# interpreting-video-features/interpreting-video-features

Hardware: AMD Instinct MI355X
Metric: clips/sec full mask-search (I3D, 16f, 300 iters) (higher is better)
Workload: dtype f32 (each operand as 3 bf16 planes = 24 significand bits, 6 MFMA passes, f32 accumulate, f32 storage); 1 GPU; I3D perturbation mask search, 300 iters, synthetic clips [32,3,16,224,224] per GPU per step (BASELINE configs[1]); init_mask + search + reverse score + Grad-CAM; iters=300, frames=16, math=bf16x6

## Files before the change

### interpreting-video-features_amd/csrc/conv3d.hip

```cpp
#include "conv_common.h"

namespace ivf {

template <int BM, int BN, int WM, int WN>
__global__ __launch_bounds__(256) void conv3d_igemm_kernel(ConvKArgs a) {
  constexpr int TM = BM / WM / 32;
  constexpr int TN = BN / WN / 32;
  constexpr int AROWS = BM / 32;
  constexpr int BROWS = BN / 32;
  static_assert(WM * WN == 4, "4 waves");
  static_assert(TM >= 1 && TN >= 1, "tile");

  __shared__ __attribute__((aligned(16))) float lds_a[BM * LDS_LD];
  __shared__ __attribute__((aligned(16))) float lds_b[BN * LDS_LD];

  const int tid = threadIdx.x;
  const int lane = tid & 63;
  const int wave = tid >> 6;
  const int wm = wave / WN, wn = wave % WN;
  const int li = lane & 31, lh = lane >> 5;

  const int tile = xcd_remap(blockIdx.x, a.mtiles * a.ntiles);
  const int mt = tile / a.ntiles;
  const int nt = tile - mt * a.ntiles;
  const int m0 = mt * BM;
  const int n0 = nt * BN;

  const int g = tid & 7;
  const int r0 = tid >> 3;

  int a_base[AROWS];
  int a_t0[AROWS], a_h0[AROWS], a_w0[AROWS];
#pragma unroll
  for (int j = 0; j < AROWS; ++j) {
    int m = m0 + r0 + 32 * j;
    if (m < a.M) {
      int wo = m % a.Wo;
      int t1 = m / a.Wo;
      int ho = t1 % a.Ho;
      int t2 = t1 / a.Ho;
      int to = t2 % a.To;
      int b = t2 / a.To;
      a_t0[j] = to * a.sT - a.pT;
      a_h0[j] = ho * a.sH - a.pH;
      a_w0[j] = wo * a.sW - a.pW;
      a_base[j] = b * a.Ti;
    } else {
      a_t0[j] = -100000;
      a_h0[j] = 0;
      a_w0[j] = 0;
      a_base[j] = 0;
    }
  }
  const float* wrow[BROWS];
#pragma unroll
  for (int j = 0; j < BROWS; ++j) {
    int n = n0 + r0 + 32 * j;
    wrow[j] = (n < a.Cout) ? a.w + (size_t)n * a.K : nullptr;
  }

  float4 ra[AROWS], rb[BROWS];
  const int khw = a.kH * a.kW;

  auto load_chunk = [&](int k0) {
    int kk = k0 + 4 * g;
    bool kvalid = kk < a.K;
    int tap = kvalid ? kk / a.Cin : 0;
    int ci = kk - tap * a.Cin;
    int kt = tap / khw;
    int rem = tap - kt * khw;
    int kh = rem / a.kW;
    int kw = rem - kh * a.kW;
#pragma unroll
    for (int j = 0; j < AROWS; ++j) {
      int ti = a_t0[j] + kt, hi = a_h0[j] + kh, wi = a_w0[j] + kw;
      bool ok = kvalid && (unsigned)ti < (unsigned)a.Ti && (unsigned)hi < (unsigned)a.Hi &&
                (unsigned)wi < (unsigned)a.Wi;
      float4 v = make_float4(0.f, 0.f, 0.f, 0.f);
      if (ok) {
        size_t pos = (size_t)((a_base[j] + ti) * a.Hi + hi) * a.Wi + wi;
        v = (a.in2 && kk >= a.K0)
                ? *reinterpret_cast<const float4*>(a.in2 + pos * a.in2_ld + a.in2_coff + (kk - a.K0))
                : *reinterpret_cast<const float4*>(a.in + pos * a.in_ld + a.in_coff + ci);
      }
      ra[j] = v;
    }
#pragma unroll
    for (int j = 0; j < BROWS; ++j) {
      float4 v = make_float4(0.f, 0.f, 0.f, 0.f);
      if (kvalid && wrow[j]) v = *reinterpret_cast<const float4*>(wrow[j] + kk);
      rb[j] = v;
    }
  };

  f32x16 acc[TM][TN];
#pragma unroll
  for (int i = 0; i < TM; ++i)
#pragma unroll
    for (int j = 0; j < TN; ++j)
#pragma unroll
      for (int r = 0; r < 16; ++r) acc[i][j][r] = 0.f;

  const int nchunks = (a.K + BK - 1) / BK;
  load_chunk(0);
  for (int c = 0; c < nchunks; ++c) {
#pragma unroll
    for (int j = 0; j < AROWS; ++j)
      *reinterpret_cast<float4*>(&lds_a[(r0 + 32 * j) * LDS_LD + 4 * g]) = ra[j];
#pragma unroll
    for (int j = 0; j < BROWS; ++j)
      *reinterpret_cast<float4*>(&lds_b[(r0 + 32 * j) * LDS_LD + 4 * g]) = rb[j];
    __syncthreads();
    if (c + 1 < nchunks) load_chunk((c + 1) * BK);

#pragma unroll
    for (int k8 = 0; k8 < BK / 8; ++k8) {
      float4 fa[TM], fb[TN];
#pragma unroll
      for (int i = 0; i < TM; ++i)
        fa[i] = *reinterpret_cast<const float4*>(
            &lds_a[(wm * (BM / WM) + i * 32 + li) * LDS_LD + k8 * 8 + 4 * lh]);
#pragma unroll
      for (int j = 0; j < TN; ++j)
        fb[j] = *reinterpret_cast<const float4*>(
            &lds_b[(wn * (BN / WN) + j * 32 + li) * LDS_LD + k8 * 8 + 4 * lh]);
#pragma unroll
      for (int i = 0; i < TM; ++i)
#pragma unroll
        for (int j = 0; j < TN; ++j) {
          acc[i][j] = __builtin_amdgcn_mfma_f32_32x32x2f32(fa[i].x, fb[j].x, acc[i][j], 0, 0, 0);
          acc[i][j] = __builtin_amdgcn_mfma_f32_32x32x2f32(fa[i].y, fb[j].y, acc[i][j], 0, 0, 0);
          acc[i][j] = __builtin_amdgcn_mfma_f32_32x32x2f32(fa[i].z, fb[j].z, acc[i][j], 0, 0, 0);
          acc[i][j] = __builtin_amdgcn_mfma_f32_32x32x2f32(fa[i].w, fb[j].w, acc[i][j], 0, 0, 0);
        }
    }
    __syncthreads();
  }

  conv_epilogue<AM_X3, TM, TN>(a, acc, [&](int row) { int m = m0 + row; return m < a.M ? m : -1; }, wm * (BM / WM),
                               n0 + wn * (BN / WN), li, lh);
}

template <int AM, int BM, int BN, int WM, int WN, bool PW>
__global__ __launch_bounds__(256) void conv3d_igemm_bf16_kernel(ConvKArgs a) {
  constexpr int NPA = OpPlanes<AM>::A, NPB = OpPlanes<AM>::B;
  constexpr int TM = BM / WM / 32;
  constexpr int TN = BN / WN / 32;
  constexpr int AROWS = BM / 32;
  constexpr int BROWS = (BN + 63) / 64;
  static_assert(WM * WN == 4 && TM >= 1 && TN >= 1, "tile");
  static_assert((NPA * BM + NPB * BN) * LDS_ROW_BF * 2 <= 64 * 1024, "static LDS");

  __shared__ __attribute__((aligned(16))) unsigned short a_pl[NPA][BM * LDS_ROW_BF];
  __shared__ __attribute__((aligned(16))) unsigned short b_pl[NPB][BN * LDS_ROW_BF];

  const int tid = threadIdx.x;
  const int lane = tid & 63;
  const int wave = tid >> 6;
  const int wm = wave / WN, wn = wave % WN;
  const int li = lane & 31, lh = lane >> 5;

  const int tile = xcd_remap(blockIdx.x, a.mtiles * a.ntiles);
  const int mt = tile / a.ntiles;
  const int nt = tile - mt * a.ntiles;
  const int m0 = mt * BM;
  const int n0 = nt * BN;

  const int g = tid & 7;
  const int r0 = perm8(tid >> 3);
  const int g2 = tid & 3;
  const int q0 = perm8(tid >> 2);

  int a_base[AROWS], a_t0[AROWS], a_h0[AROWS], a_w0[AROWS];
  size_t a_o1[AROWS], a_o2[AROWS];
#pragma unroll
  for (int j = 0; j < AROWS; ++j) {
    int m = m0 + r0 + 32 * j;
    if constexpr (PW) {
      const size_t mc = (size_t)min(m, a.M - 1);
      a_o1[j] = mc * a.in_ld + a.in_coff;
      a_o2[j] = a.in2 ? mc * a.in2_ld + a.in2_coff - a.K0 : a_o1[j];
      a_base[j] = a_t0[j] = a_h0[j] = a_w0[j] = 0;
    } else if (m < a.M) {
      int wo = m % a.Wo;
      int t1 = m / a.Wo;
      int ho = t1 % a.Ho;
      int t2 = t1 / a.Ho;
      int to = t2 % a.To;
      int b = t2 / a.To;
      a_t0[j] = to * a.sT - a.pT;
      a_h0[j] = ho * a.sH - a.pH;
      a_w0[j] = wo * a.sW - a.pW;
      a_base[j] = b * a.Ti;
      a_o1[j] = (size_t)(((long long)((a_base[j] + a_t0[j]) * a.Hi + a_h0[j]) * a.Wi + a_w0[j]) * a.in_ld + a.in_coff);
      a_o2[j] = 0;
    } else {
      a_t0[j] = -100000; a_h0[j] = 0; a_w0[j] = 0; a_base[j] = 0;
      a_o1[j] = a_o2[j] = 0;
    }
  }
  const unsigned short* wrow[BROWS];
#pragma unroll
  for (int j = 0; j < BROWS; ++j) {
    int n = n0 + q0 + 64 * j;
    wrow[j] = (q0 + 64 * j < BN && n < a.Cout) ? a.wbf + (size_t)n * a.ldw : nullptr;
  }

  float4 ra[AROWS];
  uint4 rb[NPB][BROWS];
  int d_ci, d_kw, d_kh, d_kt, s_ci, s_kw, s_kh, s_kt;
  {
    const int khw = a.kH * a.kW;
    int tap = (4 * g) / a.Cin;
    d_ci = 4 * g - tap * a.Cin;
    d_kt = tap / khw;
    int rem = tap - d_kt * khw;
    d_kh = rem / a.kW;
    d_kw = rem - d_kh * a.kW;
    tap = BK / a.Cin;
    s_ci = BK - tap * a.Cin;
    s_kt = tap / khw;
    rem = tap - s_kt * khw;
    s_kh = rem / a.kW;
    s_kw = rem - s_kh * a.kW;
  }

  auto load_chunk = [&](int k0) {
    if constexpr (PW) {
      const int kk = min(k0 + 4 * g, a.K - 4);
      const bool second = a.in2 && kk >= a.K0;
#pragma unroll
      for (int j = 0; j < AROWS; ++j)
        ra[j] = second ? load_act4<AM>(a.in2, a_o2[j] + kk) : load_act4<AM>(a.in, a_o1[j] + kk);
    } else {
      const bool kvalid = d_kt < a.kT;
      const size_t tapoff = (size_t)((long long)((d_kt * a.Hi + d_kh) * a.Wi + d_kw) * a.in_ld + d_ci);
#pragma unroll
      for (int j = 0; j < AROWS; ++j) {
        int ti = a_t0[j] + d_kt, hi = a_h0[j] + d_kh, wi = a_w0[j] + d_kw;
        bool ok = kvalid && (unsigned)ti < (unsigned)a.Ti && (unsigned)hi < (unsigned)a.Hi &&
                  (unsigned)wi < (unsigned)a.Wi;
        float4 v = make_float4(0.f, 0.f, 0.f, 0.f);
        if (ok) v = load_act4<AM>(a.in, a_o1[j] + tapoff);
        ra[j] = v;
      }
      d_ci += s_ci;
      int cw = s_kw, ch = s_kh;
      if (d_ci >= a.Cin) { d_ci -= a.Cin; ++cw; }
      d_kw += cw;
      if (d_kw >= a.kW) { d_kw -= a.kW; ++ch; }
      d_kh += ch;
      if (d_kh >= a.kH) { d_kh -= a.kH; ++d_kt; }
      d_kt += s_kt;
    }
    int kb = k0 + 8 * g2;
#pragma unroll
    for (int j = 0; j < BROWS; ++j) {
#pragma unroll
      for (int pl = 0; pl < NPB; ++pl) {
        uint4 h = make_uint4(0u, 0u, 0u, 0u);
        if (kb < a.ldw && wrow[j]) h = *reinterpret_cast<const uint4*>(wrow[j] + pl * a.w_lo_off + kb);
        rb[pl][j] = h;
      }
    }
  };

  f32x16 acc[TM][TN];
#pragma unroll
  for (int i = 0; i < TM; ++i)
#pragma unroll
    for (int j = 0; j < TN; ++j)
#pragma unroll
      for (int r = 0; r < 16; ++r) acc[i][j][r] = 0.f;

  const int nchunks = (a.K + BK - 1) / BK;
  load_chunk(0);
  for (int c = 0; c < nchunks; ++c) {
#pragma unroll
    for (int j = 0; j < AROWS; ++j)
      stage_planes<AM>(reinterpret_cast<unsigned char*>(&a_pl[0][(r0 + 32 * j) * LDS_ROW_BF + 4 * g]),
                       sizeof(a_pl[0]), ra[j]);
#pragma unroll
    for (int j = 0; j < BROWS; ++j) {
      if (q0 + 64 * j < BN) {
#pragma unroll
        for (int pl = 0; pl < NPB; ++pl) *reinterpret_cast<uint4*>(&b_pl[pl][(q0 + 64 * j) * LDS_ROW_BF + 8 * g2]) = rb[pl][j];
      }
    }
    __syncthreads();
    if (c + 1 < nchunks) load_chunk((c + 1) * BK);

#pragma unroll
    for (int ks = 0; ks < BK / 16; ++ks) {
      bf16x8 fa[TM][NPA], fb[TN][NPB];
#pragma unroll
      for (int i = 0; i < TM; ++i) {
        int off = (wm * (BM / WM) + i * 32 + li) * LDS_ROW_BF + ks * 16 + 8 * lh;
#pragma unroll
        for (int pl = 0; pl < NPA; ++pl) fa[i][pl] = *reinterpret_cast<const bf16x8*>(&a_pl[pl][off]);
      }
#pragma unroll
      for (int j = 0; j < TN; ++j) {
        int off = (wn * (BN / WN) + j * 32 + li) * LDS_ROW_BF + ks * 16 + 8 * lh;
#pragma unroll
        for (int pl = 0; pl < NPB; ++pl) fb[j][pl] = *reinterpret_cast<const bf16x8*>(&b_pl[pl][off]);
      }
#pragma unroll
      for (int i = 0; i < TM; ++i)
#pragma unroll
        for (int j = 0; j < TN; ++j) mma_planes<AM>(fa[i], fb[j], acc[i][j]);
    }
    __syncthreads();
  }
  conv_epilogue<AM, TM, TN>(a, acc, [&](int row) { int m = m0 + row; return m < a.M ? m : -1; }, wm * (BM / WM),
                            n0 + wn * (BN / WN), li, lh);
}

__device__ __forceinline__ void store_packed(float* out, int math, size_t row, int k, int ldw, size_t rows,
                                             float v) {
  if (math == 0) {
    out[row * ldw + k] = v;
  } else {
    unsigned short* o = reinterpret_cast<unsigned short*>(out);
    unsigned h = pk_bf16(v, 0.f) & 0xffffu;
    const float r1 = v - __uint_as_float(h << 16);
    unsigned l = pk_bf16(r1, 0.f) & 0xffffu;
    o[row * ldw + k] = (unsigned short)h;
    o[rows * (size_t)ldw + row * ldw + k] = (unsigned short)l;
    if (math == IVF_MATH_BF16X6)
      o[2 * rows * (size_t)ldw + row * ldw + k] = (unsigned short)(pk_bf16(r1 - __uint_as_float(l << 16), 0.f) & 0xffffu);
  }
}

__global__ void pack_fwd_kernel(const float* __restrict__ w, float* __restrict__ out, int Cout,
                                int Cin, int CinP, int taps, int ldw, int math, int row0, int rows_total) {
  size_t total = (size_t)Cout * ldw;
  for (size_t i = blockIdx.x * (size_t)blockDim.x + threadIdx.x; i < total;
       i += (size_t)gridDim.x * blockDim.x) {
    int k = i % ldw;
    int co = i / ldw;
    int ci = k % CinP;
    int tap = k / CinP;
    float v = (tap < taps && ci < Cin) ? w[((size_t)co * Cin + ci) * taps + tap] : 0.f;
    store_packed(out, math, row0 + co, k, ldw, rows_total, v);
  }
}

__global__ void pack_bwd_fused1x1_kernel(const float* __restrict__ w, const float* __restrict__ scale,
                                         float* __restrict__ out, int Cout, int Cin, int CinRows, int koff,
                                         int ktotal, int ldw, int math) {
  const int span = Cout + ((koff + Cout == ktotal) ? ldw - ktotal : 0);
  size_t total = (size_t)CinRows * span;
  for (size_t i = blockIdx.x * (size_t)blockDim.x + threadIdx.x; i < total;
       i += (size_t)gridDim.x * blockDim.x) {
    int kk = i % span;
    int ci = i / span;
    float v = (kk < Cout && ci < Cin) ? (scale ? scale[kk] : 1.f) * w[(size_t)kk * Cin + ci] : 0.f;
    store_packed(out, math, ci, koff + kk, ldw, CinRows, v);
  }
}

__global__ void pack_bwd_s1_kernel(const float* __restrict__ w, const float* __restrict__ scale,
                                   float* __restrict__ out, int Cout, int Cin, int CinRows, int kT,
                                   int kH, int kW, int ldw, int math) {
  int taps = kT * kH * kW;
  size_t total = (size_t)CinRows * ldw;
  for (size_t i = blockIdx.x * (size_t)blockDim.x + threadIdx.x; i < total;
       i += (size_t)gridDim.x * blockDim.x) {
    int k = i % ldw;
    int ci = i / ldw;
    int co = k % Cout;
    int tapf = k / Cout;
    int tap = taps - 1 - tapf;
    float v = 0.f;
    if (tapf < taps && ci < Cin) v = (scale ? scale[co] : 1.f) * w[((size_t)co * Cin + ci) * taps + tap];
    store_packed(out, math, ci, k, ldw, CinRows, v);
  }
}

struct D2SPack {
  int kT, kH, kW;
  int sT, sH, sW;
  int pT, pH, pW;
  int KT, KH, KW;
  int oT, oH, oW;
};
__global__ void pack_bwd_d2s_kernel(const float* __restrict__ w, const float* __restrict__ scale,
                                    float* __restrict__ out, int Cout, int Cin, int CinP, D2SPack p, int ldw,
                                    int math) {
  int taps = p.kT * p.kH * p.kW;
  int btaps = p.KT * p.KH * p.KW;
  size_t total = (size_t)8 * CinP * ldw;
  for (size_t i = blockIdx.x * (size_t)blockDim.x + threadIdx.x; i < total;
       i += (size_t)gridDim.x * blockDim.x) {
    int k = i % ldw;
    int n = i / ldw;
    int co = k % Cout;
    int bt = k / Cout;
    if (bt >= btaps) {
      store_packed(out, math, n, k, ldw, (size_t)8 * CinP, 0.f);
      continue;
    }
    int ci = n % CinP, par = n / CinP;
    int pt = par >> 2, ph = (par >> 1) & 1, pw = par & 1;
    int dw = bt % p.KW, dh = (bt / p.KW) % p.KH, dt = bt / (p.KW * p.KH);
    int kt = pt + p.pT - p.sT * (dt - p.oT);
    int kh = ph + p.pH - p.sH * (dh - p.oH);
    int kw = pw + p.pW - p.sW * (dw - p.oW);
    bool ok = ci < Cin && pt < p.sT && ph < p.sH && pw < p.sW && kt >= 0 && kt < p.kT && kh >= 0 &&
              kh < p.kH && kw >= 0 && kw < p.kW;
    float v = 0.f;
    if (ok) {
      int tap = (kt * p.kH + kh) * p.kW + kw;
      v = (scale ? scale[co] : 1.f) * w[((size_t)co * Cin + ci) * taps + tap];
    }
    store_packed(out, math, n, k, ldw, (size_t)8 * CinP, v);
  }
}

__global__ void bn_fold_kernel(const float* gamma, const float* beta, const float* mean,
                               const float* var, float eps, float* scale, float* shift, int C) {
  int c = blockIdx.x * blockDim.x + threadIdx.x;
  if (c < C) {
    float s = gamma[c] / sqrtf(var[c] + eps);
    scale[c] = s;
    shift[c] = beta[c] - mean[c] * s;
  }
}

template <int AM, int BM, int BN, int WM, int WN>
static void launch_bf16(ConvKArgs& a, bool pw, dim3 grid, hipStream_t s) {
  if (pw)
    hipLaunchKernelGGL((conv3d_igemm_bf16_kernel<AM, BM, BN, WM, WN, true>), grid, dim3(256), 0, s, a);
  else
    hipLaunchKernelGGL((conv3d_igemm_bf16_kernel<AM, BM, BN, WM, WN, false>), grid, dim3(256), 0, s, a);
}

template <int BM, int BN, int WM, int WN>
static int launch_variant(ConvKArgs& a, int math, hipStream_t s) {
  a.mtiles = cdiv(a.M, BM);
  a.ntiles = cdiv(a.Cout, BN);
  dim3 grid(a.mtiles * a.ntiles);
  const int cls = BM == 64 ? (BN == 64 ? 10 : 11)
                  : BN > 128 ? (BN == 256 ? 7 : (BN == 192 ? 8 : 9))
                             : IVF_CONV_IGEMM_BASE + (BN == 128 ? 0 : (BN == 64 ? 1 : 2)) + (math ? 3 : 0);
  constexpr bool wide = BN > 128 || BM == 64;
  constexpr bool fits_x6 = (3 * BM + 3 * BN) * LDS_ROW_BF * 2 <= 64 * 1024;
  if (wide && math == IVF_MATH_FP32) {
    set_error("conv3d: wide implicit-GEMM tiles exist for the split-bf16 modes only");
    return IVF_ERR_UNSUPPORTED;
  }
  if (!fits_x6 && math == IVF_MATH_BF16X6) {
    set_error("conv3d: this implicit-GEMM tile does not fit the LDS with three operand planes");
    return IVF_ERR_UNSUPPORTED;
  }
  if (math == IVF_MATH_FP32)
    prof_name(cls, "conv3d_igemm_kernel<%d,%d,%d,%d>", BM, BN, WM, WN);
  const bool pw = a.kT * a.kH * a.kW == 1 && a.sT == 1 && a.sH == 1 && a.sW == 1 && a.pT == 0 && a.pH == 0 && a.pW == 0 &&
                  a.To == a.Ti && a.Ho == a.Hi && a.Wo == a.Wi && a.K >= 4 && a.K % 4 == 0 && !a.d2s;
  if (a.in2 && !pw && math != IVF_MATH_FP32) {
    set_error("conv3d: a second input needs the plain-GEMM form (1x1x1, stride 1, no padding, K a multiple of 4)");
    return IVF_ERR_UNSUPPORTED;
  }
  if (math != IVF_MATH_FP32)
    prof_name(cls, "conv3d_igemm_bf16_kernel<%d,%d,%d,%d,%d,%s>", math == IVF_MATH_BF16X6 ? AM_X6 : (math == IVF_MATH_BF16ACT ? AM_BF16 : AM_X3),
              BM, BN, WM, WN, pw ? "true" : "false");
  const bool timed = prof_begin(s, cls);
  if (math == IVF_MATH_FP32) {
    if constexpr (!wide) hipLaunchKernelGGL((conv3d_igemm_kernel<BM, BN, WM, WN>), grid, dim3(256), 0, s, a);
  } else if (math == IVF_MATH_BF16X3) {
    launch_bf16<AM_X3, BM, BN, WM, WN>(a, pw, grid, s);
  } else if (math == IVF_MATH_BF16ACT) {
    launch_bf16<AM_BF16, BM, BN, WM, WN>(a, pw, grid, s);
  } else {
    if constexpr (fits_x6) launch_bf16<AM_X6, BM, BN, WM, WN>(a, pw, grid, s);
  }
  if (timed) prof_end(s);
  IVF_CHECK_LAUNCH();
  return IVF_OK;
}

int conv_launch(ConvKArgs& a, int math, hipStream_t s) {
  int n128 = cdiv(a.Cout, 128) * 128, n64 = cdiv(a.Cout, 64) * 64, n32 = cdiv(a.Cout, 32) * 32;
  if (n128 <= n64 && n128 <= n32) return launch_variant<128, 128, 2, 2>(a, math, s);
  if (n64 <= n32) return launch_variant<128, 64, 4, 1>(a, math, s);
  return launch_variant<128, 32, 4, 1>(a, math, s);
}

int conv_igemm_launch_variant(ConvKArgs& a, int math, int v, hipStream_t s) {
  switch (v) {
    case 0: return launch_variant<128, 128, 2, 2>(a, math, s);
    case 1: return launch_variant<128, 64, 4, 1>(a, math, s);
    case 2: return launch_variant<128, 32, 4, 1>(a, math, s);
    case 3: return launch_variant<128, 256, 4, 1>(a, math, s);
    case 4: return launch_variant<128, 192, 4, 1>(a, math, s);
    case 5: return launch_variant<128, 160, 4, 1>(a, math, s);
    case 6: return launch_variant<64, 64, 2, 2>(a, math, s);
    case 7: return launch_variant<64, 128, 2, 2>(a, math, s);
  }
  set_error("conv3d: unknown implicit-GEMM variant %d", v);
  return IVF_ERR_BAD_ARG;
}

static inline int pack_ldw(int K, int math) { return math ? (K + 7) / 8 * 8 : K; }
static inline size_t pack_floats(size_t rows, int ldw, int math) {
  return math ? (rows * ldw * math_planes(math) + 1) / 2 : rows * ldw;
}

static void bwd_span(int k, int st, int pad, int* K, int* off) {
  if (st == 1) { *K = k; *off = k - 1 - pad; return; }
  int lo_num = pad - (k - 1);
  int dlo = lo_num >= 0 ? (lo_num + st - 1) / st : -((-lo_num) / st);
  int dhi = (st - 1 + pad) / st;
  *K = dhi - dlo + 1;
  *off = -dlo;
}

static int check_desc(const ivf_conv3d_desc* d) {
  IVF_CHECK_ARG(d != nullptr, "conv3d: null descriptor");
  IVF_CHECK_ARG(d->B > 0 && d->Ti > 0 && d->Hi > 0 && d->Wi > 0, "conv3d: bad input dims");
  IVF_CHECK_ARG(d->Cin > 0 && d->Cin % 4 == 0, "conv3d: Cin (%d) must be a positive multiple of 4", d->Cin);
  const int cin_first = d->in2 ? d->K0 : d->Cin;
  IVF_CHECK_ARG(d->in_ld % 4 == 0 && d->in_coff % 4 == 0 && d->in_coff + cin_first <= d->in_ld,
                "conv3d: input channel window [%d,+%d) must be 4-aligned inside ld %d", d->in_coff,
                cin_first, d->in_ld);
  IVF_CHECK_ARG(d->Cout > 0 && d->out_coff >= 0, "conv3d: bad Cout");
  IVF_CHECK_ARG(d->kT > 0 && d->kH > 0 && d->kW > 0 && d->sT > 0 && d->sH > 0 && d->sW > 0,
                "conv3d: bad kernel/stride");
  IVF_CHECK_ARG(d->To > 0 && d->Ho > 0 && d->Wo > 0, "conv3d: bad output dims");
  long long in_elems = (long long)d->B * d->Ti * d->Hi * d->Wi * d->in_ld;
  IVF_CHECK_ARG(in_elems < (1ll << 40), "conv3d: input too large");
  IVF_CHECK_ARG((long long)d->B * d->To * d->Ho * d->Wo < (1ll << 31) &&
                    (long long)d->B * d->Ti * d->Hi * d->Wi < (1ll << 31),
                "conv3d: position count exceeds int32");
  return IVF_OK;
}

}

using namespace ivf;

extern "C" int ivf_conv3d(const ivf_conv3d_desc* d, const float* in, const float* w_packed,
                          const float* scale, const float* shift, const float* relu_mask,
                          float* out, ivf_stream_t stream) {
  IVF_PROPAGATE(check_desc(d));
  IVF_CHECK_ARG(in && w_packed && out, "conv3d: null pointer");
  ConvKArgs a;
  a.in = in; a.w = w_packed; a.out = out; a.scale = scale; a.shift = shift; a.mask = relu_mask;
  a.B = d->B; a.Ti = d->Ti; a.Hi = d->Hi; a.Wi = d->Wi; a.Cin = d->Cin; a.in_ld = d->in_ld;
  a.in_coff = d->in_coff;
  a.To = d->To; a.Ho = d->Ho; a.Wo = d->Wo; a.Cout = d->Cout; a.out_ld = d->out_ld;
  a.out_coff = d->out_coff; a.mask_ld = d->mask_ld; a.mask_coff = d->mask_coff;
  a.kT = d->kT; a.kH = d->kH; a.kW = d->kW; a.sT = d->sT; a.sH = d->sH; a.sW = d->sW;
  a.pT = d->pT; a.pH = d->pH; a.pW = d->pW;
  a.K = d->kT * d->kH * d->kW * d->Cin;
  a.M = d->B * d->To * d->Ho * d->Wo;
  a.in2 = d->in2; a.in2_ld = d->in2_ld; a.in2_coff = d->in2_coff; a.K0 = d->K0;
  if (d->in2) {
    IVF_CHECK_ARG(d->kT * d->kH * d->kW == 1, "conv3d: a second input is only defined for 1x1x1 convs");
    IVF_CHECK_ARG(d->K0 > 0 && d->K0 < d->Cin && d->K0 % 4 == 0 && d->in2_ld % 4 == 0 && d->in2_coff % 4 == 0 &&
                      d->in2_coff + (d->Cin - d->K0) <= d->in2_ld,
                  "conv3d: second-input channel window must be 4-aligned inside its row");
  }
  a.out2 = d->out2; a.out2_ld = d->out2_ld; a.out2_coff = d->out2_coff; a.N0 = d->N0;
  if (d->out2) {
    IVF_CHECK_ARG(!d->accumulate && relu_mask == nullptr && !d->d2s,
                  "conv3d: a second output window is a forward-epilogue feature (no accumulate / relu_mask / d2s)");
    IVF_CHECK_ARG(d->N0 > 0 && d->N0 < d->Cout && d->out2_coff >= 0 && d->out2_coff + (d->Cout - d->N0) <= d->out2_ld &&
                      d->out_coff + d->N0 <= d->out_ld,
                  "conv3d: output windows [0,N0) / [N0,Cout) must fit their rows");
    IVF_CHECK_ARG(d->variant == IVF_CONV_AUTO || (d->variant >= IVF_CONV_IGEMM_BASE && d->variant < IVF_CONV_PIX4),
                  "conv3d: a second output window is served by the implicit-GEMM tiles only");
  }
  a.gbo = d->gate_out; a.gbo2 = d->gate_out2; a.gbi = d->gate_in;
  a.gbo_ld = d->gate_out_ld; a.gbo_coff = d->gate_out_coff; a.gbo2_ld = d->gate_out2_ld;
  a.gbi_ld = d->gate_in_ld; a.gbi_coff = d->gate_in_coff;
  if (d->gate_out || d->gate_out2 || d->gate_in) {
    IVF_CHECK_ARG(!d->d2s && (d->Cout & 7) == 0 && (d->out_ld & 3) == 0 && (d->out_coff & 3) == 0,
                  "conv3d: 1-bit gates need Cout %% 8 == 0 and 4-aligned output rows (the 16-byte epilogue)");
    IVF_CHECK_ARG(d->variant != IVF_CONV_PIX4, "conv3d: the pix4 kernel does not record 1-bit gates");
    IVF_CHECK_ARG(!d->out2 || ((d->N0 | d->out2_ld | d->out2_coff) & 3) == 0, "conv3d: 1-bit gates with out2 need 4-aligned windows");
  }
  if (d->gate_out || d->gate_out2) {
    IVF_CHECK_ARG(!d->accumulate && relu_mask == nullptr && !d->gate_in,
                  "conv3d: gate_out / gate_out2 are forward-epilogue records (no accumulate / relu_mask / gate_in)");
    IVF_CHECK_ARG(!d->gate_out || ((d->gate_out_coff & 7) == 0 && d->gate_out_ld > 0), "conv3d: gate_out window must be 8-aligned");
    IVF_CHECK_ARG(!d->gate_out2 || (d->out2 && (d->N0 & 7) == 0 && (d->out2_coff & 7) == 0 && d->gate_out2_ld > 0),
                  "conv3d: gate_out2 needs out2 with 8-aligned N0 / out2_coff");
  }
  if (d->gate_in)
    IVF_CHECK_ARG(relu_mask == nullptr && (d->gate_in_coff & 3) == 0 && d->gate_in_ld > 0,
                  "conv3d: gate_in replaces relu_mask (give one of them) and needs a 4-aligned channel offset");
  IVF_CHECK_ARG(d->math >= IVF_MATH_FP32 && d->math <= IVF_MATH_BF16ACT, "conv3d: math must be one of IVF_MATH_* (0..3)");
  if (d->math == IVF_MATH_BF16ACT) {
    IVF_CHECK_ARG(!(d->d2s && (d->accumulate || d->relu)), "conv3d: bf16act depth-to-space output is a plain fp32 store");
  }
  a.ldw = pack_ldw(a.K, d->math);
  a.wbf = reinterpret_cast<const unsigned short*>(w_packed);
  a.w_lo_off = (long)d->Cout * a.ldw;
  a.relu = d->relu; a.accumulate = d->accumulate; a.d2s = d->d2s;
  a.dT = d->dT; a.dH = d->dH; a.dW = d->dW; a.dC = d->dC;
  a.bsT = d->bsT; a.bsH = d->bsH; a.bsW = d->bsW;
  if (d->d2s) {
    IVF_CHECK_ARG(relu_mask == nullptr, "conv3d: relu_mask unsupported with depth-to-space");
    IVF_CHECK_ARG(d->bsT >= 1 && d->bsT <= 2 && d->bsH >= 1 && d->bsH <= 2 && d->bsW >= 1 && d->bsW <= 2,
                  "conv3d: block strides must be 1 or 2");
    IVF_CHECK_ARG(d->Cout % 8 == 0 && d->Cout <= 32, "conv3d: depth-to-space needs Cout = 8 * Cpad <= 32");
    IVF_CHECK_ARG(d->dT > 0 && d->dH > 0 && d->dW > 0 && d->dC > 0 && d->dC <= d->Cout / 8,
                  "conv3d: bad depth-to-space dims");
    IVF_CHECK_ARG(d->out_coff + d->dC <= d->out_ld, "conv3d: d2s output window outside ld");
  } else if (!d->out2) {
    IVF_CHECK_ARG(d->out_coff + d->Cout <= d->out_ld, "conv3d: output window outside ld");
  }
  if (d->math == 0) IVF_CHECK_ARG(a.ldw == a.K, "conv3d: internal ldw");
  const bool bf = d->math != IVF_MATH_FP32;
  const bool act_stem = d->math == IVF_MATH_BF16ACT && conv_pix4_supported(a);
  const bool act_d2s = d->math == IVF_MATH_BF16ACT && d->d2s;
  if (d->variant != IVF_CONV_AUTO) {
    if (d->variant == IVF_CONV_PIX4) {
      IVF_CHECK_ARG(bf && conv_pix4_supported(a), "conv3d: pix4 variant needs a split-bf16 mode, 4-channel pixels, stride (1|2,2,2), k <= 7");
      return conv_pix4_launch(a, d->math, IVF_CONV_PIX4, (hipStream_t)stream);
    }
    IVF_CHECK_ARG(!act_stem, "conv3d: bf16act reads fp32 pixels through the pix4 kernel only");
    if (d->variant >= IVF_CONV_HALO_BASE) {
      IVF_CHECK_ARG(bf && conv_halo_supported(a), "conv3d: halo variant needs a split-bf16 mode, stride 1, k in 2..4");
      return conv_halo_launch_variant(a, d->math, d->variant - IVF_CONV_HALO_BASE, (hipStream_t)stream);
    }
    IVF_CHECK_ARG(!act_d2s, "conv3d: bf16act depth-to-space (fp32 output) is served by the LDS-halo kernel only");
// ... 133 lines not shown
```

### interpreting-video-features_amd/csrc/conv_common.h

```cpp
#pragma once
#include "ivf_common.h"

namespace ivf {

typedef float f32x16 __attribute__((ext_vector_type(16)));
typedef float f32x4 __attribute__((ext_vector_type(4)));

constexpr int BK = 32;
constexpr int LDS_LD = BK + 4;

struct ConvKArgs {
  const float* in;
  const float* w;
  float* out;
  const float* scale;
  const float* shift;
  const float* mask;
  int B, Ti, Hi, Wi, Cin, in_ld, in_coff;
  int To, Ho, Wo, Cout, out_ld, out_coff;
  int mask_ld, mask_coff;
  int kT, kH, kW, sT, sH, sW, pT, pH, pW;
  int K, M;
  int relu, accumulate, d2s;
  int dT, dH, dW, dC;
// ... 178 lines not shown
            int t = a.bsT * tb + pt, h = a.bsH * hb + ph, w = a.bsW * wb + pw;
            if (t >= a.dT || h >= a.dH || w >= a.dW) continue;
            size_t off = ((size_t)((b * a.dT + t) * a.dH + h) * a.dW + w) * a.out_ld + a.out_coff;
            float4 o = make_float4(v0, v1, v2, v3);
            if (a.accumulate) {
              float4 old = *reinterpret_cast<const float4*>(a.out + off);
              o.x += old.x; o.y += old.y; o.z += old.z; o.w += old.w;
            }
            if (a.relu) { o.x = fmaxf(o.x, 0.f); o.y = fmaxf(o.y, 0.f); o.z = fmaxf(o.z, 0.f); o.w = fmaxf(o.w, 0.f); }
            if (a.dC == 4 && (a.out_ld & 3) == 0 && (a.out_coff & 3) == 0) {
              *reinterpret_cast<float4*>(a.out + off) = o;
            } else {
              float ov[4] = {o.x, o.y, o.z, o.w};
              for (int q = 0; q < a.dC && q < 4; ++q) a.out[off + q] = ov[q];
            }
          } else {
            if (!nvalid || c >= a.dC || m < 0) continue;
            int wb = m % a.Wo;
            int t1 = m / a.Wo;
            int hb = t1 % a.Ho;
            int t2 = t1 / a.Ho;
            int tb = t2 % a.To;
            int b = t2 / a.To;
            int t = a.bsT * tb + pt, h = a.bsH * hb + ph, w = a.bsW * wb + pw;
            if (t >= a.dT || h >= a.dH || w >= a.dW) continue;
            size_t off = ((size_t)((b * a.dT + t) * a.dH + h) * a.dW + w) * a.out_ld + a.out_coff + c;
            if (a.accumulate) v += a.out[off];
            if (a.relu) v = v > 0.f ? v : 0.f;
            a.out[off] = v;
          }
        }
      }
    }
    return;
  }
  const bool vec_ok = (a.Cout & 3) == 0 && (a.out_ld & 3) == 0 && (a.out_coff & 3) == 0 && (col_base & 3) == 0 &&
                      (!a.mask || (((a.mask_ld | a.mask_coff) & 3) == 0)) &&
                      (!a.out2 || (((a.N0 | a.out2_ld | a.out2_coff) & 3) == 0));
  if (vec_ok) {
    const int q = li & 3;
#pragma unroll
    for (int j = 0; j < TN; ++j) {
      const int n = col_base + j * 32 + li;
      const int nq = n & ~3;
      const bool nvalid = nq < a.Cout;
      const float sc = (a.scale && nvalid) ? a.scale[n] : 1.f;
      const float sh = (a.shift && nvalid) ? a.shift[n] : 0.f;
      const bool second = a.out2 != nullptr && nq >= a.N0;
      float* const obase = second ? a.out2 : a.out;
      const size_t ocol = second ? (size_t)(a.out2_coff + (nq - a.N0)) : (size_t)(a.out_coff + nq);
      const size_t oldim = second ? (size_t)a.out2_ld : (size_t)a.out_ld;
#pragma unroll
      for (int i = 0; i < TM; ++i) {
        const int rbase = row_base + i * 32 + 4 * lh;
        float4 old4[4], gate4[4];
        unsigned gnib[4];
        int mrow[4];
#pragma unroll
        for (int g = 0; g < 4; ++g) {
          const int m = mrow[g] = rowmap(rbase + q + 8 * g);
          const bool ok = nvalid && m >= 0;
          old4[g] = (a.accumulate && ok) ? ep_ld4_raw<OB>(obase, ocol + (size_t)m * oldim) : make_float4(0.f, 0.f, 0.f, 0.f);
          gate4[g] = (a.mask && ok) ? ep_ld4_raw<OB>(a.mask, (size_t)m * a.mask_ld + a.mask_coff + nq)
                                    : (OB ? make_float4(__uint_as_float(0x3f803f80u), __uint_as_float(0x3f803f80u), 0.f, 0.f)
                                          : make_float4(1.f, 1.f, 1.f, 1.f));
          unsigned gb = 0xffu;
          if (a.gbi && ok) gb = a.gbi[(size_t)m * a.gbi_ld + ((a.gbi_coff + nq) >> 3)];
          gnib[g] = gb;
        }
#pragma unroll
        for (int g = 0; g < 4; ++g) gnib[g] = (gnib[g] >> ((a.gbi_coff + nq) & 4)) & 15u;
#pragma unroll
        for (int g = 0; g < 4; ++g) {
          float v[4];
#pragma unroll
          for (int k = 0; k < 4; ++k) v[k] = acc[i][j][4 * g + k] * sc + sh;
          quad_transpose4(v, q);
          const int m = mrow[g];
          if (a.gbo || a.gbo2) {
            unsigned nib = 0u;
#pragma unroll
            for (int k = 0; k < 4; ++k) {
              float t = v[k];
              if (a.relu) t = t > 0.f ? t : 0.f;
              nib |= (t > 0.f ? 1u : 0u) << k;
            }
            const unsigned hi = (unsigned)__shfl_down((int)nib, 4, 64);
            if (nvalid && m >= 0 && ((li >> 2) & 1) == 0) {
              if (second) {
                if (a.gbo2) a.gbo2[(size_t)m * a.gbo2_ld + ((a.out2_coff + nq - a.N0) >> 3)] = (unsigned char)(nib | (hi << 4));
              } else if (a.gbo) {
                a.gbo[(size_t)m * a.gbo_ld + ((a.gbo_coff + nq) >> 3)] = (unsigned char)(nib | (hi << 4));
              }
            }
          }
          if (!nvalid || m < 0) continue;
          const float4 oc = ep_cvt4<OB>(old4[g]), gc = ep_cvt4<OB>(gate4[g]);
          const float o4[4] = {oc.x, oc.y, oc.z, oc.w};
          const float g4[4] = {gc.x, gc.y, gc.z, gc.w};
#pragma unroll
          for (int k = 0; k < 4; ++k) {
            float t = v[k] + o4[k];
            if (a.relu) t = t > 0.f ? t : 0.f;
            if (!(g4[k] > 0.f) || !((gnib[g] >> k) & 1u)) t = 0.f;
            v[k] = t;
          }
          ep_st4<OB>(obase, ocol + (size_t)m * oldim, v[0], v[1], v[2], v[3]);
        }
      }
    }
    return;
  }
#pragma unroll
  for (int j = 0; j < TN; ++j) {
    const int n = col_base + j * 32 + li;
    const bool nvalid = n < a.Cout;
    const float sc = (a.scale && nvalid) ? a.scale[n] : 1.f;
    const float sh = (a.shift && nvalid) ? a.shift[n] : 0.f;
    const bool second = a.out2 != nullptr && n >= a.N0;
    float* const obase = second ? a.out2 : a.out;
    const size_t ocol = second ? (size_t)(a.out2_coff + (n - a.N0)) : (size_t)(a.out_coff + n);
    const size_t oldim = second ? (size_t)a.out2_ld : (size_t)a.out_ld;
#pragma unroll
    for (int i = 0; i < TM; ++i) {
      const int rbase = row_base + i * 32 + 4 * lh;
#pragma unroll
      for (int half = 0; half < 2; ++half) {
        float old[8], gate[8];
        int mrow[8];
#pragma unroll
        for (int q = 0; q < 8; ++q) {
          const int r = half * 8 + q;
          const int m = mrow[q] = rowmap(rbase + (r & 3) + 8 * (r >> 2));
          const bool ok = nvalid && m >= 0;
          old[q] = (a.accumulate && ok) ? ep_ld1<OB>(obase, ocol + (size_t)m * oldim) : 0.f;
          gate[q] = (a.mask && ok) ? ep_ld1<OB>(a.mask, (size_t)m * a.mask_ld + a.mask_coff + n) : 1.f;
        }
#pragma unroll
        for (int q = 0; q < 8; ++q) {
          const int m = mrow[q];
          if (!nvalid || m < 0) continue;
          float v = acc[i][j][half * 8 + q] * sc + sh + old[q];
          if (a.relu) v = v > 0.f ? v : 0.f;
          if (!(gate[q] > 0.f)) v = 0.f;
          ep_st1<OB>(obase, ocol + (size_t)m * oldim, v);
        }
      }
    }
  }
}

int conv_launch(ConvKArgs& a, int math, hipStream_t s);
int conv_igemm_launch_variant(ConvKArgs& a, int math, int v, hipStream_t s);
int conv_halo_supported(const ConvKArgs& a);
int conv_halo_launch(ConvKArgs& a, int math, hipStream_t s);
int conv_halo_num_variants();
int conv_halo_launch_variant(ConvKArgs& a, int math, int v, hipStream_t s);
int conv_pix4_supported(const ConvKArgs& a);
int conv_pix4_launch(ConvKArgs& a, int math, int variant_id, hipStream_t s);
static inline int math_planes(int math) { return math == IVF_MATH_BF16X6 ? 3 : (math == IVF_MATH_FP32 ? 0 : 2); }

}
```

Measured before the change: 3.979 clips/s.

## Add dedicated pointwise conv kernel with double-buffered swizzled LDS and shape picker

```diff
diff --git a/interpreting-video-features_amd/csrc/conv3d.hip b/interpreting-video-features_amd/csrc/conv3d.hip
--- a/interpreting-video-features_amd/csrc/conv3d.hip
+++ b/interpreting-video-features_amd/csrc/conv3d.hip
@@ -141,7 +141,7 @@
                                n0 + wn * (BN / WN), li, lh);
 }
 
-template <int AM, int BM, int BN, int WM, int WN, bool PW>
+template <int AM, int BM, int BN, int WM, int WN>
 __global__ __launch_bounds__(256) void conv3d_igemm_bf16_kernel(ConvKArgs a) {
   constexpr int NPA = OpPlanes<AM>::A, NPB = OpPlanes<AM>::B;
   constexpr int TM = BM / WM / 32;
@@ -172,16 +172,11 @@
   const int q0 = perm8(tid >> 2);
 
   int a_base[AROWS], a_t0[AROWS], a_h0[AROWS], a_w0[AROWS];
-  size_t a_o1[AROWS], a_o2[AROWS];
+  size_t a_o1[AROWS];
 #pragma unroll
   for (int j = 0; j < AROWS; ++j) {
     int m = m0 + r0 + 32 * j;
-    if constexpr (PW) {
-      const size_t mc = (size_t)min(m, a.M - 1);
-      a_o1[j] = mc * a.in_ld + a.in_coff;
-      a_o2[j] = a.in2 ? mc * a.in2_ld + a.in2_coff - a.K0 : a_o1[j];
-      a_base[j] = a_t0[j] = a_h0[j] = a_w0[j] = 0;
-    } else if (m < a.M) {
+    if (m < a.M) {
       int wo = m % a.Wo;
       int t1 = m / a.Wo;
       int ho = t1 % a.Ho;
@@ -193,10 +188,9 @@
       a_w0[j] = wo * a.sW - a.pW;
       a_base[j] = b * a.Ti;
       a_o1[j] = (size_t)(((long long)((a_base[j] + a_t0[j]) * a.Hi + a_h0[j]) * a.Wi + a_w0[j]) * a.in_ld + a.in_coff);
-      a_o2[j] = 0;
     } else {
       a_t0[j] = -100000; a_h0[j] = 0; a_w0[j] = 0; a_base[j] = 0;
-      a_o1[j] = a_o2[j] = 0;
+      a_o1[j] = 0;
     }
   }
   const unsigned short* wrow[BROWS];
@@ -226,13 +220,7 @@
   }
 
   auto load_chunk = [&](int k0) {
-    if constexpr (PW) {
-      const int kk = min(k0 + 4 * g, a.K - 4);
-      const bool second = a.in2 && kk >= a.K0;
-#pragma unroll
-      for (int j = 0; j < AROWS; ++j)
-        ra[j] = second ? load_act4<AM>(a.in2, a_o2[j] + kk) : load_act4<AM>(a.in, a_o1[j] + kk);
-    } else {
+    {
       const bool kvalid = d_kt < a.kT;
       const size_t tapoff = (size_t)((long long)((d_kt * a.Hi + d_kh) * a.Wi + d_kw) * a.in_ld + d_ci);
 #pragma unroll
@@ -429,11 +417,8 @@
 }
 
 template <int AM, int BM, int BN, int WM, int WN>
-static void launch_bf16(ConvKArgs& a, bool pw, dim3 grid, hipStream_t s) {
-  if (pw)
-    hipLaunchKernelGGL((conv3d_igemm_bf16_kernel<AM, BM, BN, WM, WN, true>), grid, dim3(256), 0, s, a);
-  else
-    hipLaunchKernelGGL((conv3d_igemm_bf16_kernel<AM, BM, BN, WM, WN, false>), grid, dim3(256), 0, s, a);
+static void launch_bf16(ConvKArgs& a, dim3 grid, hipStream_t s) {
+  hipLaunchKernelGGL((conv3d_igemm_bf16_kernel<AM, BM, BN, WM, WN>), grid, dim3(256), 0, s, a);
 }
 
 template <int BM, int BN, int WM, int WN>
@@ -462,18 +447,19 @@
     set_error("conv3d: a second input needs the plain-GEMM form (1x1x1, stride 1, no padding, K a multiple of 4)");
     return IVF_ERR_UNSUPPORTED;
   }
+  if (pw && math != IVF_MATH_FP32) return conv_pw_launch(a, math, BM, cls, s);
   if (math != IVF_MATH_FP32)
-    prof_name(cls, "conv3d_igemm_bf16_kernel<%d,%d,%d,%d,%d,%s>", math == IVF_MATH_BF16X6 ? AM_X6 : (math == IVF_MATH_BF16ACT ? AM_BF16 : AM_X3),
-              BM, BN, WM, WN, pw ? "true" : "false");
+    prof_name(cls, "conv3d_igemm_bf16_kernel<%d,%d,%d,%d,%d>", math == IVF_MATH_BF16X6 ? AM_X6 : (math == IVF_MATH_BF16ACT ? AM_BF16 : AM_X3),
+              BM, BN, WM, WN);
   const bool timed = prof_begin(s, cls);
   if (math == IVF_MATH_FP32) {
     if constexpr (!wide) hipLaunchKernelGGL((conv3d_igemm_kernel<BM, BN, WM, WN>), grid, dim3(256), 0, s, a);
   } else if (math == IVF_MATH_BF16X3) {
-    launch_bf16<AM_X3, BM, BN, WM, WN>(a, pw, grid, s);
+    launch_bf16<AM_X3, BM, BN, WM, WN>(a, grid, s);
   } else if (math == IVF_MATH_BF16ACT) {
-    launch_bf16<AM_BF16, BM, BN, WM, WN>(a, pw, grid, s);
+    launch_bf16<AM_BF16, BM, BN, WM, WN>(a, grid, s);
   } else {
-    if constexpr (fits_x6) launch_bf16<AM_X6, BM, BN, WM, WN>(a, pw, grid, s);
+    if constexpr (fits_x6) launch_bf16<AM_X6, BM, BN, WM, WN>(a, grid, s);
   }
   if (timed) prof_end(s);
   IVF_CHECK_LAUNCH();
diff --git a/interpreting-video-features_amd/csrc/conv3d_pointwise.hip b/interpreting-video-features_amd/csrc/conv3d_pointwise.hip
--- /dev/null
+++ b/interpreting-video-features_amd/csrc/conv3d_pointwise.hip
@@ -0,0 +1,217 @@
+#include "conv_common.h"
+
+namespace ivf {
+
+constexpr int PW_ROW_BYTES = BK * 2;
+
+__device__ __forceinline__ int pw_sw(int r, int p) { return r * PW_ROW_BYTES + ((p ^ ((r >> 2) & 3)) << 4); }
+
+template <int AM, int BM, int BN>
+struct PwLds {
+  static constexpr int A_PLANE = BM * PW_ROW_BYTES, B_PLANE = BN * PW_ROW_BYTES;
+  static constexpr int BUF = OpPlanes<AM>::A * A_PLANE + OpPlanes<AM>::B * B_PLANE;
+  static constexpr int BYTES = 2 * BUF;
+};
+
+template <int AM, int BM, int BN, int WM, int WN>
+__global__ __launch_bounds__(64 * WM * WN) void conv3d_pointwise_kernel(ConvKArgs a) {
+  constexpr int NPA = OpPlanes<AM>::A, NPB = OpPlanes<AM>::B;
+  constexpr int NT = 64 * WM * WN;
+  constexpr int TM = BM / WM / 32, TN = BN / WN / 32;
+  constexpr int AIT = (BM * 8 + NT - 1) / NT;
+  constexpr int BIT = (BN * 4 + NT - 1) / NT;
+  using L = PwLds<AM, BM, BN>;
+  static_assert(TM >= 1 && TN >= 1 && BM == TM * WM * 32 && BN == TN * WN * 32, "tile");
+  static_assert(L::BYTES <= 160 * 1024, "LDS");
+
+  __shared__ __attribute__((aligned(16))) unsigned char lds[L::BYTES];
+
+  const int tid = threadIdx.x;
+  const int lane = tid & 63;
+  const int wave = tid >> 6;
+  const int wm = wave / WN, wn = wave % WN;
+  const int li = lane & 31, lh = lane >> 5;
+
+  const int tile = xcd_remap(blockIdx.x, a.mtiles * a.ntiles);
+  const int mt = tile / a.ntiles;
+  const int nt = tile - mt * a.ntiles;
+  const int m0 = mt * BM;
+  const int n0 = nt * BN;
+
+  int a_g[AIT], a_dst[AIT];
+  size_t a_o1[AIT], a_o2[AIT];
+#pragma unroll
+  for (int j = 0; j < AIT; ++j) {
+    const int i = (tid + j * NT) % (BM * 8);
+    const int r = i >> 3, g = i & 7;
+    const size_t mc = (size_t)min(m0 + r, a.M - 1);
+    a_g[j] = 4 * g;
+    a_dst[j] = pw_sw(r, g >> 1) + (g & 1) * 8;
+    a_o1[j] = mc * a.in_ld + a.in_coff;
+    a_o2[j] = a.in2 ? mc * a.in2_ld + a.in2_coff - a.K0 : a_o1[j];
+  }
+  const float* const in2 = a.in2 ? a.in2 : a.in;
+  const int k_second = a.in2 ? a.K0 : 0x7fffffff;
+  int b_g[BIT], b_dst[BIT];
+  const unsigned short* wrow[BIT];
+#pragma unroll
+  for (int j = 0; j < BIT; ++j) {
+    const int i = (tid + j * NT) % (BN * 4);
+    const int q = i >> 2, g2 = i & 3;
+    b_g[j] = 8 * g2;
+    b_dst[j] = pw_sw(q, g2);
+    wrow[j] = a.wbf + (size_t)min(n0 + q, a.Cout - 1) * a.ldw;
+  }
+
+  auto load_a = [&](float4 (&ra)[AIT], int k0) {
+#pragma unroll
+    for (int j = 0; j < AIT; ++j) {
+      const int kk = min(k0 + a_g[j], a.K - 4);
+      const bool second = kk >= k_second;
+      ra[j] = load_act4<AM>(second ? in2 : a.in, (second ? a_o2[j] : a_o1[j]) + kk);
+    }
+  };
+  auto load_b = [&](uint4 (&rb)[NPB][BIT], int k0) {
+#pragma unroll
+    for (int j = 0; j < BIT; ++j) {
+      const int kb = k0 + b_g[j];
+      const bool ok = kb < a.ldw;
+      const unsigned short* p = wrow[j] + (ok ? kb : 0);
+#pragma unroll
+      for (int pl = 0; pl < NPB; ++pl) {
+        const uint4 h = *reinterpret_cast<const uint4*>(p + pl * a.w_lo_off);
+        rb[pl][j] = ok ? h : make_uint4(0u, 0u, 0u, 0u);
+      }
+    }
+  };
+  auto stage = [&](unsigned char* buf, const float4 (&ra)[AIT], const uint4 (&rb)[NPB][BIT]) {
+#pragma unroll
+    for (int j = 0; j < AIT; ++j) stage_planes<AM>(buf + a_dst[j], L::A_PLANE, ra[j]);
+    unsigned char* const bb = buf + NPA * L::A_PLANE;
+#pragma unroll
+    for (int j = 0; j < BIT; ++j)
+#pragma unroll
+      for (int pl = 0; pl < NPB; ++pl) *reinterpret_cast<uint4*>(bb + pl * L::B_PLANE + b_dst[j]) = rb[pl][j];
+  };
+
+  f32x16 acc[TM][TN];
+#pragma unroll
+  for (int i = 0; i < TM; ++i)
+#pragma unroll
+    for (int j = 0; j < TN; ++j)
+#pragma unroll
+      for (int r = 0; r < 16; ++r) acc[i][j][r] = 0.f;
+
+  const int col_base = n0 + wn * (BN / WN);
+  const int tn_live = min(TN, max(0, (a.Cout - col_base + 31) / 32));
+
+  float4 ra1[AIT], ra2[AIT];
+  uint4 rb[NPB][BIT];
+  const int nchunks = (a.K + BK - 1) / BK;
+  load_a(ra1, 0);
+  load_b(rb, 0);
+  stage(lds, ra1, rb);
+  load_b(rb, BK);
+  load_a(ra1, BK);
+  load_a(ra2, 2 * BK);
+  __syncthreads();
+  for (int c = 0; c < nchunks; ++c) {
+    unsigned char* const cur = lds + (c & 1) * L::BUF;
+    stage(lds + ((c + 1) & 1) * L::BUF, ra1, rb);
+    load_b(rb, (c + 2) * BK);
+#pragma unroll
+    for (int j = 0; j < AIT; ++j) ra1[j] = ra2[j];
+    load_a(ra2, (c + 3) * BK);
+
+    const unsigned char* const ab = cur;
+    const unsigned char* const bb = cur + NPA * L::A_PLANE;
+#pragma unroll
+    for (int ks = 0; ks < BK / 16; ++ks) {
+      bf16x8 fa[TM][NPA];
+#pragma unroll
+      for (int i = 0; i < TM; ++i) {
+        const int off = pw_sw(wm * (BM / WM) + i * 32 + li, ks * 2 + lh);
+#pragma unroll
+        for (int pl = 0; pl < NPA; ++pl) fa[i][pl] = *reinterpret_cast<const bf16x8*>(ab + pl * L::A_PLANE + off);
+      }
+#pragma unroll
+      for (int j = 0; j < TN; ++j) {
+        if (j < tn_live) {
+          bf16x8 fb[NPB];
+          const int off = pw_sw(wn * (BN / WN) + j * 32 + li, ks * 2 + lh);
+#pragma unroll
+          for (int pl = 0; pl < NPB; ++pl) fb[pl] = *reinterpret_cast<const bf16x8*>(bb + pl * L::B_PLANE + off);
+#pragma unroll
+          for (int i = 0; i < TM; ++i) mma_planes<AM>(fa[i], fb, acc[i][j]);
+        }
+      }
+    }
+    __syncthreads();
+  }
+  conv_epilogue<AM, TM, TN>(a, acc, [&](int row) { int m = m0 + row; return m < a.M ? m : -1; }, wm * (BM / WM),
+                            col_base, li, lh);
+}
+
+struct PwShape { int bm, bn, wm, wn; };
+static const PwShape kPwShapes[] = {
+    {128, 32, 4, 1},  {128, 64, 4, 1}, {128, 128, 4, 2}, {128, 192, 4, 2}, {128, 256, 2, 4}, {128, 288, 4, 3},
+    {64, 32, 2, 1},   {64, 64, 2, 2},  {64, 128, 2, 2},  {64, 256, 2, 4},
+};
+constexpr int kPwNumShapes = sizeof(kPwShapes) / sizeof(kPwShapes[0]);
+
+template <int AM, int BM, int BN, int WM, int WN>
+static void pw_launch_one(ConvKArgs& a, hipStream_t s) {
+  hipLaunchKernelGGL((conv3d_pointwise_kernel<AM, BM, BN, WM, WN>), dim3(a.mtiles * a.ntiles), dim3(64 * WM * WN), 0, s, a);
+}
+template <int AM>
+static void pw_launch_shape(ConvKArgs& a, int shape, hipStream_t s) {
+  switch (shape) {
+    case 0: return pw_launch_one<AM, 128, 32, 4, 1>(a, s);
+    case 1: return pw_launch_one<AM, 128, 64, 4, 1>(a, s);
+    case 2: return pw_launch_one<AM, 128, 128, 4, 2>(a, s);
+    case 3: return pw_launch_one<AM, 128, 192, 4, 2>(a, s);
+    case 4: return pw_launch_one<AM, 128, 256, 2, 4>(a, s);
+    case 5: return pw_launch_one<AM, 128, 288, 4, 3>(a, s);
+    case 6: return pw_launch_one<AM, 64, 32, 2, 1>(a, s);
+    case 7: return pw_launch_one<AM, 64, 64, 2, 2>(a, s);
+    case 8: return pw_launch_one<AM, 64, 128, 2, 2>(a, s);
+    case 9: return pw_launch_one<AM, 64, 256, 2, 4>(a, s);
+  }
+}
+
+int conv_pw_pick_shape(int M, int Cout, int bm) {
+  int best = -1, best_cost = 0, best_wgs = 0;
+  for (int i = 0; i < kPwNumShapes; ++i) {
+    const PwShape& p = kPwShapes[i];
+    if (p.bm != bm) continue;
+    const int nt = cdiv(Cout, p.bn);
+    const int cost = nt * (p.bn + 48);
+    const int wgs = cdiv(M, p.bm) * nt;
+    bool take;
+    if (best < 0) take = true;
+    else if (best_wgs >= 512 && wgs >= 512) take = cost <= best_cost;
+    else if (best_wgs >= 512) take = false;
+    else if (wgs >= 512) take = true;
+    else take = wgs > best_wgs || (wgs == best_wgs && cost <= best_cost);
+    if (take) { best = i; best_cost = cost; best_wgs = wgs; }
+  }
+  return best;
+}
+
+int conv_pw_launch(ConvKArgs& a, int math, int bm, int cls, hipStream_t s) {
+  const int shape = conv_pw_pick_shape(a.M, a.Cout, bm);
+  const PwShape& p = kPwShapes[shape];
+  a.mtiles = cdiv(a.M, p.bm);
+  a.ntiles = cdiv(a.Cout, p.bn);
+  const int am = math == IVF_MATH_BF16X6 ? AM_X6 : (math == IVF_MATH_BF16ACT ? AM_BF16 : AM_X3);
+  prof_name(cls, "conv3d_pointwise_kernel<%d,%d,%d,%d,%d>", am, p.bm, p.bn, p.wm, p.wn);
+  const bool timed = prof_begin(s, cls);
+  if (am == AM_X6) pw_launch_shape<AM_X6>(a, shape, s);
+  else if (am == AM_BF16) pw_launch_shape<AM_BF16>(a, shape, s);
+  else pw_launch_shape<AM_X3>(a, shape, s);
+  if (timed) prof_end(s);
+  IVF_CHECK_LAUNCH();
+  return IVF_OK;
+}
+
+}
diff --git a/interpreting-video-features_amd/csrc/conv_common.h b/interpreting-video-features_amd/csrc/conv_common.h
--- a/interpreting-video-features_amd/csrc/conv_common.h
+++ b/interpreting-video-features_amd/csrc/conv_common.h
@@ -354,6 +354,8 @@
 
 int conv_launch(ConvKArgs& a, int math, hipStream_t s);
 int conv_igemm_launch_variant(ConvKArgs& a, int math, int v, hipStream_t s);
+int conv_pw_launch(ConvKArgs& a, int math, int bm, int cls, hipStream_t s);
+int conv_pw_pick_shape(int M, int Cout, int bm);
 int conv_halo_supported(const ConvKArgs& a);
 int conv_halo_launch(ConvKArgs& a, int math, hipStream_t s);
 int conv_halo_num_variants();
```

Result: slower. 3.879 clips/s (-2.5%).
